# yoshihikoueno/DNNCancerAnnotator

Measured on AMD Instinct MI355X. Metric: MRI slices/sec (fwd+bwd) unet 512x512 bs=8, higher is better.
Workload: dtype f32; 1 GPU; configs/unet.yaml train step (fwd + weighted BCE + bwd + Adam), batch 8 x 512x512x1 per GPU, f32, random-init weights; global_batch=8, parallelism=dp1, kernels=tuned, communicator=False

## Files before the change

### dnncancerannotator_amd/csrc/kernels_mfma.hip

```cpp
#include <stdio.h>
#include <stdlib.h>

#include "fast.h"
#include "kernels.h"
#include "tconv2_dev.h"

namespace dnnca {

typedef float f32x4 __attribute__((ext_vector_type(4)));

static constexpr int TH = 8;
static constexpr int NBUCKET = kPgBuckets;

template <int C, int TW>
struct TG {
    static constexpr int HL = (C + 3) / 4 * 4;
    static constexpr int LEAD = HL - C;
    static constexpr int LS = (LEAD + (TW + 2) * C + 3 + 3) / 4 * 4;
    static constexpr int LS4 = LS / 4;
    static constexpr int N4 = (TH + 2) * LS4;
    static constexpr int npf(int nt) { return (N4 + nt - 1) / nt; }
};

__device__ __forceinline__ void lds_barrier() { asm volatile("s_waitcnt lgkmcnt(0)\n\ts_barrier" ::: "memory"); }
// ... 317 lines not shown
        }
    }
}

__device__ __forceinline__ unsigned long long stamp() {
    unsigned long long t;
    asm volatile("s_memtime %0\n\ts_waitcnt lgkmcnt(0)" : "=s"(t)::"memory");
    return t;
}
#ifdef DNNCA_TUNING
#define STAMP(i)                                                                                        \
    do {                                                                                                \
        if (p.stamps && wave == 0 && lane == 0 && it < 4) p.stamps[((size_t)blockIdx.x * 4 + it) * 8 + (i)] = stamp(); \
    } while (0)
#define STAMP_END(i)                                                                                    \
    do {                                                                                                \
        if (p.stamps && wave == 0 && lane == 0) p.stamps[((size_t)blockIdx.x * 4 + 3) * 8 + (i)] = stamp(); \
    } while (0)
#define DBG_FLAGS(p) ((p).dbg)
#else
#define STAMP(i) do { } while (0)
#define STAMP_END(i) do { } while (0)
#define DBG_FLAGS(p) 0
#endif

struct BwdArgs {
    const float* dz;
    const float* x[2];
    const float* bmat;
    float* dx[2];
    float* slabs[2];
    int acc[2];
    int mask[2];
    int B, H, W;
    int tiles_x, tiles_y;
    float alpha;
    const float* pf_y;
    const float* pf_dpool;
    const unsigned char* pf_idx;
    float pf_alpha;
    const float* tc_in;
    float* tc_din;
    const float* tc_w;
    float* tc_slabs;
    int tc_mask;
    float tc_alpha;
    int dbg;
    unsigned long long* stamps;
};

template <int C, int NSRC, int CO>
struct BW {
    static constexpr int Gw = 12 / CO;
    static constexpr int TW = 32 * Gw;
    static constexpr int CTOT = NSRC * C;
    static constexpr int NPASS = CTOT <= 12 ? 1 : NSRC;
    static constexpr int COd = CTOT / NPASS;
    static constexpr int Gd = (COd == 3 || COd == 6 || COd == 12) ? 12 / COd : (COd == 1 ? 4 : 1);
    static constexpr int WRd = (Gd + 2) * CO, SRd = (WRd + 3) / 4, KSd = 3 * SRd;
    static constexpr int MTX = TW / (16 * Gd);
    static constexpr int WRw = (Gw + 2) * C;
    static constexpr int MROWS = 3 * WRw + 1;
    static constexpr int MT = (MROWS + 15) / 16;
    using TGg = TG<CO, TW>;
    using TGx = TG<C, TW>;
    static constexpr int STAGE4 = TGg::N4 + NSRC * TGx::N4;
    static constexpr int RED4 = NSRC * MT * 256;
    static constexpr int LDS4 = STAGE4 > RED4 ? STAGE4 : RED4;
};

#define DNNCA_DPP_ADD(v, ctrl, rmask) \
    (v) += __builtin_bit_cast(float, __builtin_amdgcn_update_dpp(0, __builtin_bit_cast(int, (v)), (ctrl), (rmask), 0xf, true))
__device__ __forceinline__ float wave_total_l63(float v) {
    DNNCA_DPP_ADD(v, 0x118, 0xf);
    DNNCA_DPP_ADD(v, 0x114, 0xf);
    DNNCA_DPP_ADD(v, 0x112, 0xf);
    DNNCA_DPP_ADD(v, 0x111, 0xf);
    DNNCA_DPP_ADD(v, 0x142, 0xa);
    DNNCA_DPP_ADD(v, 0x143, 0xc);
    return v;
}
__device__ __forceinline__ int slab_index(int mrow, int n);

template <int C, int NSRC, int CO, bool DGRAD, int NT, bool VW = false, bool PF = false, bool TCF = false, bool TCM = false, bool CW = false>
__global__ __launch_bounds__(NT, (VW && NSRC == 1) ? 4 : 1) void k_pgbwd(BwdArgs p) {
    constexpr int NW = NT / 64;
    static_assert(!CW || TCF, "CW is the counted-wait form of the TCF kernel");
    static_assert(!TCF || (VW && NSRC == 2 && C == 3 && CO == 3), "TCF rides in the two-source 3-channel VW kernel");
    static_assert(!TCM || (!VW && !PF && !TCF && NSRC == 2 && DGRAD && C == CO && (C == 6 || C == 12)), "TCM: two-source C -> C conv");
    static_assert(!PF || (NSRC == 1 && C == CO && DGRAD && !VW), "PF: single-source C -> C conv with data gradient");
    static_assert(!VW || (C == 3 && CO == 3 && NT == 512 && DGRAD), "VW: 3 -> 3 channels, eight waves, with data gradient");
    constexpr int NWD = VW ? NW / 2 : NW;
    using Wc = BW<C, NSRC, CO>;
    using TGg = typename Wc::TGg;
    using TGx = typename Wc::TGx;
    constexpr int TW = Wc::TW, Gw = Wc::Gw, Gd = Wc::Gd, COd = Wc::COd, NPASS = Wc::NPASS, SRd = Wc::SRd, KSd = Wc::KSd;
    constexpr int MT = Wc::MT, WRw = Wc::WRw, LSg = TGg::LS, LSx = TGx::LS, Nw = Gw * CO, Nd = Gd * COd;
    static_assert(TW % (16 * Gd) == 0, "tile width must hold whole dgrad M-tiles");
    constexpr int MAIN4 = Wc::LDS4;
    constexpr int PFR = TH / 2 + 2, PFW = Wc::TW / 2 + 2, PFLEAD = (4 - CO % 4) % 4;
    constexpr int PFLS = (PFLEAD + PFW * CO + 3) / 4 * 4, PFN4 = PF ? PFR * PFLS / 4 : 0, PFLI = PFLS / 4, PFNI = PF ? PFR * PFLI : 0;
    constexpr int TCF4 = TCF ? TH * 4 * 24 + 18 : 0;
    constexpr int CIt = 12, KA = 2 * C, KTt = 4 * C, KS1 = KA / 4, MBt = (KTt + 15) / 16;
    constexpr int LWt = Wc::TW / 2, NLP = (TH / 2) * LWt, ROWF = Wc::TW * C;
    constexpr int DT4 = TCM ? TH * ROWF / 4 : 0, XLT4 = TCM ? NLP * CIt / 4 : 0, TCW4 = TCM ? KTt * CIt / 4 : 0;
    static_assert(!TCM || (XLT4 <= NT && LWt % 16 == 0), "TCM: one staging slot per thread, whole M-tiles per input row");
    constexpr int TCM0 = MAIN4 + NW * 48 + 1 + PFN4 + (PFNI + 3) / 4 + TCF4;
    constexpr int DTF = TCM0 * 4, XLTF = DTF + DT4 * 4, TCWF = XLTF + XLT4 * 4;
    constexpr bool TLDS = TCM && C == 12;
    constexpr int TSUM0 = TCM0 + DT4 + XLT4 + TCW4, TSUM4 = TLDS ? NW * MBt * 64 : 0;
    constexpr int DUMP4 = CW ? NT : 0;
    __shared__ float4 lds4[TSUM0 + TSUM4 + DUMP4];
    float* orow = reinterpret_cast<float*>(lds4 + MAIN4) + (threadIdx.x >> 6) * 192;
    float4* dta4 = lds4 + MAIN4 + NW * 48 + 1 + PFN4 + (PFNI + 3) / 4;
    float* tcw = reinterpret_cast<float*>(dta4 + TH * 4 * 24);
    float* pf_dp = reinterpret_cast<float*>(lds4 + MAIN4 + NW * 48 + 1);
    unsigned* pf_ix = reinterpret_cast<unsigned*>(lds4 + MAIN4 + NW * 48 + 1 + PFN4);
    constexpr int NPS = PF ? (PFN4 + NT - 1) / NT : 1;
    static_assert(PFNI == PFN4, "the two pooled tiles have the same number of staging slots");

    const int tid = threadIdx.x, lane = tid & 63, wave = tid >> 6;
    const int m16 = lane & 15, q = lane >> 4, n = m16;
    const int ntiles = p.tiles_x * p.tiles_y * p.B;
    const bool xcd_map = (ntiles & 7) == 0 && (gridDim.x & 7) == 0;

    float* cst = reinterpret_cast<float*>(lds4 + MAIN4 + NW * 48);
    if (threadIdx.x == 0) { cst[0] = 1.0f; cst[1] = 0.0f; }
    if constexpr (TCF) {
        if (threadIdx.x < 72) tcw[threadIdx.x] = p.tc_w[threadIdx.x];
    }
    float tacc[TCF ? 72 : 1], tbias[TCF ? 3 : 1];
#pragma unroll
    for (int i = 0; i < (TCF ? 72 : 1); ++i) tacc[i] = 0.f;
#pragma unroll
    for (int i = 0; i < (TCF ? 3 : 1); ++i) tbias[i] = 0.f;
    const float* ldsf = reinterpret_cast<const float*>(lds4);
    constexpr int CST1 = (MAIN4 + NW * 48) * 4, CST0 = CST1 + 1;
    int offA[MT], stepA[MT];
#pragma unroll
    for (int t = 0; t < MT; ++t) {
        const int mrow = 16 * t + m16;
        if (mrow < 3 * WRw) {
            const int dy = mrow / WRw, j = mrow - dy * WRw;
            offA[t] = dy * LSx + TGx::LEAD + j + q * (Gw * C);
            stepA[t] = 4 * Gw * C;
        } else {
            offA[t] = mrow == 3 * WRw ? CST1 : CST0;
            stepA[t] = 0;
        }
    }
    f32x4 acc[NSRC][MT];
#pragma unroll
    for (int s = 0; s < NSRC; ++s)
#pragma unroll
        for (int t = 0; t < MT; ++t) acc[s][t] = f32x4{0.f, 0.f, 0.f, 0.f};
    constexpr int NWACC = !VW ? 1 : (NSRC == 2 ? 84 : 27);
    float wacc[NWACC];
#pragma unroll
    for (int i = 0; i < NWACC; ++i) wacc[i] = 0.f;

    f32x4 tacc2[TCM ? MBt : 1];
    if constexpr (TCM) {
        if (tid < TCW4) lds4[TCM0 + DT4 + XLT4 + tid] = reinterpret_cast<const float4*>(p.tc_w)[tid];
        if constexpr (TLDS) {
#pragma unroll
            for (int t = 0; t < MBt; ++t) lds4[TSUM0 + (wave * MBt + t) * 64 + lane] = make_float4(0.f, 0.f, 0.f, 0.f);
        }
#pragma unroll
        for (int t = 0; t < MBt; ++t) {
            tacc2[t] = f32x4{0.f, 0.f, 0.f, 0.f};
        }
    }
    if (VW && wave < NWD) __builtin_amdgcn_s_setprio(2);
    float breg[DGRAD ? NPASS * KSd : 1];
    if (DGRAD) {
#pragma unroll
        for (int s = 0; s < NPASS * KSd; ++s) breg[s] = p.bmat[s * 64 + lane];
    }
    const int dxp = n / COd, cod = n % COd;

    float4 preg[TGg::npf(NT)];
    float4 prex[NSRC][TGx::npf(NT)];
    TileMap<CO, TW, NT> mpg;
    TileMap<C, TW, NT> mpx;
    mpg.init(tid, p.W * CO / 4);
    mpx.init(tid, p.W * C / 4);
    float4 prey[PF ? TGg::npf(NT) : 1];
    float4 predp[NPS];
    unsigned preix[NPS];
    auto pf_issue = [&](int b, int x0, int y0) {
        if constexpr (PF) {
            (void)tile_issue<CO, TW, NT>(prey, mpg, p.pf_y, b, x0, y0, p.B, p.H, p.W);
            const int Hp = p.H >> 1, Wp = p.W >> 1, rowf = Wp * CO;
#pragma unroll
            for (int k = 0; k < NPS; ++k) {
                const int id = tid + k * NT;
                const int r = id / PFLI, c4 = id - r * PFLI;
                const int gy = (y0 >> 1) - 1 + r, gf = ((x0 >> 1) - 1) * CO - PFLEAD + 4 * c4;
                const bool ok = id < PFN4 && (unsigned)gy < (unsigned)Hp && gf >= 0 && gf < rowf;
                const size_t off = ok ? ((size_t)b * Hp + gy) * rowf + gf : 0;
                predp[k] = *reinterpret_cast<const float4*>(p.pf_dpool + off);
                if (!ok) predp[k] = make_float4(0.f, 0.f, 0.f, 0.f);
                preix[k] = *reinterpret_cast<const unsigned*>(p.pf_idx + off);
                if (!ok) preix[k] = 0xffffffffu;
            }
        }
    };
    auto pf_commit_pooled = [&]() {
        if constexpr (PF) {
#pragma unroll
            for (int k = 0; k < NPS; ++k) {
                const int id = tid + k * NT;
                if (id < PFN4) {
                    reinterpret_cast<float4*>(pf_dp)[id] = predp[k];
                    pf_ix[id] = preix[k];
                }
            }
        }
    };
    auto pf_transform = [&](unsigned ok) {
        if constexpr (PF) {
            const unsigned char* ixb = reinterpret_cast<const unsigned char*>(pf_ix);
#pragma unroll
            for (int k = 0; k < TGg::npf(NT); ++k) {
                const int r = mpg.row[k], c4 = mpg.c4[k];
                float g[4] = {preg[k].x, preg[k].y, preg[k].z, preg[k].w};
                const float yv[4] = {prey[k].x, prey[k].y, prey[k].z, prey[k].w};
                const bool in = (ok >> k) & 1u;
#pragma unroll
                for (int e = 0; e < 4; ++e) {
                    const int f = 4 * c4 + e - TGg::LEAD;
                    if (in && f >= 0 && f < (TW + 2) * CO) {
                        const int px = f / CO, ch = f - px * CO;
                        const int pr = ((r - 1) >> 1) + 1, pc = ((px - 1) >> 1) + 1;
                        const unsigned pos = (((unsigned)(r - 1) & 1u) << 1) | ((unsigned)(px - 1) & 1u);
                        const int o = PFLEAD + pc * CO + ch;
                        const float dp = ixb[pr * PFLS + o] == pos ? pf_dp[pr * PFLS + o] : 0.f;
                        g[e] = (g[e] + dp) * (yv[e] > 0.f ? 1.0f : p.pf_alpha);
                    }
                }
                preg[k] = make_float4(g[0], g[1], g[2], g[3]);
            }
        }
    };
    unsigned okg = 0, okx = 0;
    auto decode = [&](int t, int& b, int& x0, int& y0) {
        if (xcd_map) t = (t & 7) * (ntiles >> 3) + (t >> 3);
        const int bx = t % p.tiles_x, by = (t / p.tiles_x) % p.tiles_y;
        b = t / (p.tiles_x * p.tiles_y);
        x0 = bx * TW;
        y0 = by * TH;
    };
    int tile = blockIdx.x;
    int it = 0;
    (void)it;
    STAMP(6);
    if (tile < ntiles) {
        int b, x0, y0;
        decode(tile, b, x0, y0);
        okg = tile_issue<CO, TW, NT>(preg, mpg, p.dz, b, x0, y0, p.B, p.H, p.W);
        pf_issue(b, x0, y0);
#pragma unroll
        for (int s = 0; s < NSRC; ++s) okx = tile_issue<C, TW, NT>(prex[s], mpx, p.x[s], b, x0, y0, p.B, p.H, p.W);
    }
    if (DGRAD) {
        asm volatile("s_waitcnt vmcnt(0)" ::: "memory");
#pragma unroll
        for (int s = 0; s < NPASS * KSd; ++s) asm volatile("" : "+v"(breg[s]));
    }

    if constexpr (!CW) {
#define PGBWD_ROLE 0
#include "pgbwd_tiles.h"
#undef PGBWD_ROLE
    } else if (wave < NWD) {
#define PGBWD_ROLE 1
#include "pgbwd_tiles.h"
#undef PGBWD_ROLE
    } else {
#define PGBWD_ROLE 2
#include "pgbwd_tiles.h"
#undef PGBWD_ROLE
        __builtin_amdgcn_s_waitcnt(PG_WAIT_VMCNT0);
    }

    STAMP_END(5);
    if constexpr (VW) {
        float* red = reinterpret_cast<float*>(lds4);
        __syncthreads();
        if (wave >= NWD) {
            const int wv = wave - NWD;
#pragma unroll
            for (int i = 0; i < NWACC; ++i) {
                const float t = wave_total_l63(wacc[i]);
                if (lane == 63 && (NSRC == 2 || wv < 3 || i < 3)) red[NSRC == 2 ? wv * 84 + i : wv * 27 + i] = t;
            }
        } else if constexpr (TCF) {
#pragma unroll
            for (int i = 0; i < 72; ++i) {
                const float t = wave_total_l63(tacc[i]);
                if (lane == 63) red[4 * 84 + wave * 75 + i] = t;
            }
#pragma unroll
            for (int i = 0; i < 3; ++i) {
                const float t = wave_total_l63(tbias[i]);
                if (lane == 63) red[4 * 84 + wave * 75 + 72 + i] = t;
            }
        }
        __syncthreads();
        if constexpr (TCF) {
            if (tid < 75) {
                const float* r2 = red + 4 * 84;
                const float v = (r2[tid] + r2[75 + tid]) + (r2[150 + tid] + r2[225 + tid]);
                const int mrow = tid < 72 ? tid / 6 : tid - 72, col = tid < 72 ? tid % 6 : 6;
                atomicAdd(p.tc_slabs + (size_t)(blockIdx.x % NBUCKET) * 256 + slab_index(mrow, col), v);
            }
        }
        const int bucket = blockIdx.x % NBUCKET;
        for (int i = tid; i < NSRC * 84; i += NT) {
            const int s = i / 84, e = i - s * 84;
            const float v = NSRC == 2 ? red[(2 * s) * 84 + e] + red[(2 * s + 1) * 84 + e] : red[e];
            const int mrow = e < 81 ? (e / 27) * WRw + (e / 3) % 9 : 3 * WRw, co = e < 81 ? e % 3 : e - 81;
            atomicAdd(p.slabs[s] + (size_t)bucket * (MT * 256) + slab_index(mrow, co), v);
        }
        return;
    }
    float* red = reinterpret_cast<float*>(lds4);
    constexpr int PER = NSRC * MT * 256;
    if (NW == 8) {
        if (wave >= 4) {
#pragma unroll
            for (int s = 0; s < NSRC; ++s)
#pragma unroll
                for (int t = 0; t < MT; ++t)
#pragma unroll
                    for (int r = 0; r < 4; ++r) red[(wave - 4) * PER + ((s * MT + t) * 4 + r) * 64 + lane] = acc[s][t][r];
        }
        __syncthreads();
        if (wave < 4) {
#pragma unroll
            for (int s = 0; s < NSRC; ++s)
#pragma unroll
                for (int t = 0; t < MT; ++t)
#pragma unroll
                    for (int r = 0; r < 4; ++r) acc[s][t][r] += red[wave * PER + ((s * MT + t) * 4 + r) * 64 + lane];
        }
        __syncthreads();
    }
    if (wave < 4) {
#pragma unroll
        for (int s = 0; s < NSRC; ++s)
#pragma unroll
            for (int t = 0; t < MT; ++t)
// ... 818 lines not shown
    const int TW = 32 * (12 / CO);
    a.tiles_x = (a.W + TW - 1) / TW;
    a.tiles_y = (a.H + TH - 1) / TH;
    const int ntiles = a.tiles_x * a.tiles_y * B;
    const double bytes = out_bytes + (o.need_din ? 2 : 1) * in_bytes;
    const double fl = (o.need_din ? 2 : 1) * flops;
    if (m->step.pool_fold.conv == &o) {
        auto f3 = pl.first3.find(&o);
        if (f3 != pl.first3.end()) {
            Op* c0 = f3->second;
            const Op& pool = *m->step.pool_fold.pool;
            m->step.pool_fold.conv = nullptr;
            FirstArgs f{};
            f.dskip = o.out.g.p; f.y1 = o.out.d.p;
            f.dpool = pool.out.g.p; f.idx = pool.pool_idx;
            f.x1 = o.inA.d.p; f.xin = c0->inA.d.p;
            f.w = m->p + o.w_off;
            f.pf_alpha = pool.mask_alpha;
            f.mask = o.maskA; f.mask_alpha = o.mask_alpha;
            f.slabs1 = a.slabs[0];
            f.slabs0 = pl.slabs + pl.folds[pl.wslot.find({c0, 0})->second].slab_off;
            f.B = B; f.H = a.H; f.W = a.W;
            const StripGrid sg = strip_grid(B, a.H, a.W, 2048);
            f.nstrips = sg.nstrips; f.nchunks = sg.nchunks;
            const double npx = (double)B * a.H * a.W;
            LAUNCH(m, "first3_bwd", 4.0 * npx * 20.5, 2.0 * npx * (162 + 30),
                   hipLaunchKernelGGL((k_first3<2, 40>), dim3(sg.nblocks), dim3(256), 0, m->stream, f));
            m->step.first_done = c0;
            return true;
        }
    }
    if (!sw.no_bwd3v && o.need_din && C == 3 && CO == 3 && NS == 1 && !o.accA && a.W % 128 == 0 && a.H % TH == 0) {
        const bool pf = m->step.pool_fold.conv == &o;
        double pb = 0.0;
        if (pf) {
            const Op& pool = *m->step.pool_fold.pool;
            m->step.pool_fold.conv = nullptr;
            a.pf_y = o.out.d.p;
            a.pf_dpool = pool.out.g.p;
            a.pf_idx = pool.pool_idx;
            a.pf_alpha = pool.mask_alpha;
            pb = 4.0 * (2 * (double)B * o.out.d.H * o.out.d.W * CO + 2 * (double)B * pool.out.d.H * pool.out.d.W * CO);
        }
        const float* wts = m->p + o.w_off;
        if (a.stamps && pf != sw.stamps_pf) a.stamps = nullptr;
        if (pf) {
            const int g = pg_grid<k_bwd3v<true>, 256>(m, ntiles);
            LAUNCH(m, "bwd3v_pool_3x1_3", bytes + pb, fl, hipLaunchKernelGGL(k_bwd3v<true>, dim3(g), dim3(256), 0, m->stream, a, wts));
        } else {
            const int g = pg_grid<k_bwd3v<false>, 256>(m, ntiles);
#ifdef DNNCA_TUNING
            if (sw.abl == 1) {
                LAUNCH(m, "bwd3v_3x1_3", bytes, fl, hipLaunchKernelGGL((k_bwd3v<false, 1>), dim3(g), dim3(256), 0, m->stream, a, wts));
                return true;
            }
#endif
            LAUNCH(m, "bwd3v_3x1_3", bytes, fl, hipLaunchKernelGGL(k_bwd3v<false>, dim3(g), dim3(256), 0, m->stream, a, wts));
        }
        return true;
    }
    if (m->step.pool_fold.conv == &o) {
        const Op& pool = *m->step.pool_fold.pool;
        m->step.pool_fold.conv = nullptr;
        a.pf_y = o.out.d.p;
        a.pf_dpool = pool.out.g.p;
        a.pf_idx = pool.pool_idx;
        a.pf_alpha = pool.mask_alpha;
        const double pb = 4.0 * (2 * (double)B * o.out.d.H * o.out.d.W * CO + 2 * (double)B * pool.out.d.H * pool.out.d.W * CO);
#define PFX(c)                                                                                                          \
        if (C == c) {                                                                                                   \
            const int g = pg_grid<k_pgbwd<c, 1, c, true, 512, false, true>>(m, ntiles);                                 \
            LAUNCH(m, "pgbwd_pool_" #c "x1_" #c, bytes + pb, fl,                                                        \
                   hipLaunchKernelGGL((k_pgbwd<c, 1, c, true, 512, false, true>), dim3(g), dim3(512), 0, m->stream, a)); \
            return true;                                                                                                \
        }
        PFX(3) PFX(6) PFX(12)
#undef PFX
        return false;
    }
    if (!sw.no_vw && o.need_din && C == 3 && CO == 3 && NS == 2) {
        if (Op* tc = sw.no_tcf ? nullptr : riding_tconv(m, pl, o, 6, a)) {
            const double tb = 4.0 * ((double)B * a.H * a.W * 3 + (double)B * (a.H / 2) * (a.W / 2) * 6);
            if (!sw.pgbwd_old && !a.acc[1] && (size_t)a.H * a.W * 3 * 4 < (size_t)PG_NOWHERE) {
                const int g = pg_grid<k_pgbwd<3, 2, 3, true, 512, true, false, true, false, true>>(m, ntiles);
                LAUNCH(m, "pgbwd_tc_3x2_3", bytes + 2 * tb, fl + 4.0 * B * a.H * a.W * 3 * 6,
                       hipLaunchKernelGGL((k_pgbwd<3, 2, 3, true, 512, true, false, true, false, true>), dim3(g), dim3(512), 0, m->stream, a));
            } else {
                const int g = pg_grid<k_pgbwd<3, 2, 3, true, 512, true, false, true>>(m, ntiles);
                LAUNCH(m, "pgbwd_tc_3x2_3", bytes + 2 * tb, fl + 4.0 * B * a.H * a.W * 3 * 6,
                       hipLaunchKernelGGL((k_pgbwd<3, 2, 3, true, 512, true, false, true>), dim3(g), dim3(512), 0, m->stream, a));
            }
            m->step.tconv_done = tc;
            return true;
        }
        const int g = pg_grid<k_pgbwd<3, 2, 3, true, 512, true>>(m, ntiles);
        LAUNCH(m, "pgbwd_3x2_3", bytes, fl, hipLaunchKernelGGL((k_pgbwd<3, 2, 3, true, 512, true>), dim3(g), dim3(512), 0, m->stream, a));
        return true;
    }
    if (o.need_din && NS == 2 && C == CO && (C == 6 || C == 12) && !sw.no_tcm) {
        if (Op* tc = riding_tconv(m, pl, o, 12, a)) {
            const double tb = 4.0 * ((double)B * a.H * a.W * C + (double)B * (a.H / 2) * (a.W / 2) * 12);
            const double tfl = 4.0 * B * a.H * a.W * C * 12;
#define TCMX(c)                                                                                                         \
            if (C == c) {                                                                                               \
                const int g = pg_grid<k_pgbwd<c, 2, c, true, 512, false, false, false, true>>(m, ntiles);               \
                LAUNCH(m, "pgbwd_tc_" #c "x2_" #c, bytes + 2 * tb, fl + tfl,                                            \
                       hipLaunchKernelGGL((k_pgbwd<c, 2, c, true, 512, false, false, false, true>), dim3(g), dim3(512), 0, m->stream, a)); \
                m->step.tconv_done = tc;                                                                                     \
                return true;                                                                                            \
            }
            TCMX(6) TCMX(12)
#undef TCMX
        }
    }
#define X(c, ns, co)                                                                                            \
    if (C == c && NS == ns && CO == co) {                                                                       \
        if (o.need_din) {                                                                                       \
            const int g = pg_grid<k_pgbwd<c, ns, co, true, 512>>(m, ntiles);                                    \
            LAUNCH(m, "pgbwd_" #c "x" #ns "_" #co, bytes, fl,                                                   \
                   hipLaunchKernelGGL((k_pgbwd<c, ns, co, true, 512>), dim3(g), dim3(512), 0, m->stream, a));   \
        } else {                                                                                                \
            const int g = pg_grid<k_pgbwd<c, ns, co, false, 512>>(m, ntiles);                                   \
            LAUNCH(m, "pgbwd_w_" #c "x" #ns "_" #co, bytes, fl,                                                 \
                   hipLaunchKernelGGL((k_pgbwd<c, ns, co, false, 512>), dim3(g), dim3(512), 0, m->stream, a));  \
        }                                                                                                       \
        return true;                                                                                            \
    }
    CONV_SHAPES(X)
#undef X
    return false;
}

bool fast_pool_fold(Model* m, Op& pool, Op& conv) {
    if (m->sw.no_pool_fold || pool.type != OP_POOL || pool.k != 2 || !pool.pool_idx_valid || !(pool.pool_idx || m->dry)) return false;
    if (!pool.accA || !pool.maskA || pool.mask_alpha != 0.f) return false;
    if (!conv_supported(m, conv) || conv.inB.d.C || !conv.need_din || conv.out.d.p != pool.inA.d.p || !conv.premasked) return false;
    const int C = conv.inA.d.C, CO = conv.out.d.C;
    if (C != CO || !(C == 3 || C == 6 || C == 12)) return false;
    const int TW = 32 * (12 / CO);
    if (!dense(pool.out.g) || !dense(pool.out.d)) return false;
    if ((conv.out.d.W % TW || conv.out.d.H % TH) && !pg_find(m).first3.count(&conv)) return false;
    pool.pool_idx_valid = false;
    m->step.pool_fold.conv = &conv;
    m->step.pool_fold.pool = &pool;
    return true;
}

bool fast_head_in_conv_possible(Model* m) {
    if (m->ops.size() < 2 || !m->head_defer_ok) return false;
    const Op& head = m->ops.back();
    const Op& o = m->ops[m->ops.size() - 2];
    if (head.type != OP_HEAD || !conv_supported(m, o)) return false;
    return o.inA.d.C == 3 && !o.inB.d.C && o.out.d.C == 3 && head.inA.d.p == o.out.d.p && head.inA.d.C == 3 && dense(head.inA.d);
}

template <typename A>
static void head_args(A& a, const Model* m, const Op& head, const float* y, const dnnca_loss_cfg& cfg, float gscale, double n_label) {
    a.hy = y;
    a.hw = m->p + head.w_off; a.hb = m->p + head.b_off;
    a.hpartials = m->head_partials;
    a.hscalars = m->scalars;
    a.hlabel_part = m->step.label_part_valid ? m->label_part : nullptr;
    a.hlabel_nblk = m->step.label_part_nblk;
    a.hcfg = cfg;
    a.hn_label = n_label;
    a.hgscale = gscale;
    a.hmask = head.maskA; a.halpha = head.mask_alpha;
}
static void head_launched(Model* m, const Op& head, int nblocks) {
// ... 253 lines not shown
```

### dnncancerannotator_amd/csrc/model.h

```cpp
#pragma once
#include <initializer_list>
#include <map>
#include <string>
#include <vector>

#include "common.h"
#include "kernels.h"

typedef struct ncclComm* ncclComm_t;

namespace dnnca {

struct OptChunk;

struct T {
    View d, g;
};

inline T tslice(const T& t, int c0, int c) { return T{slice(t.d, c0, c), slice(t.g, c0, c)}; }

enum OpType { OP_CONV = 0, OP_BN, OP_POOL, OP_TCONV, OP_HEAD, OP_JOIN };

struct Op {
    OpType type;
    std::string name;
    T inA, inB, out;
    int64_t w_off = -1, b_off = -1;
    int64_t mm_off = -1, mv_off = -1;
    float alpha = -1.f;
    int k = 0;
    float* nogamma_sum = nullptr;
    bool mean_ready = false;
    bool need_din = true;
    bool accA = false, accB = false;
    bool maskA = false, maskB = false, premasked = false;
    float mask_alpha = 0.f;
    float* coef = nullptr;
    double* ws = nullptr;
    int fused_stats_rows = 0;
    bool elided = false;
    const Op* pool_grad = nullptr;
    bool pool_grad_acc = false;
    bool bwd_sums_rode = false;
    int src_bn[2] = {-1, -1};
    std::vector<int> out_readers;
    unsigned char* pool_idx = nullptr;
    bool pool_idx_valid = false;
};

struct ParamInfo {
    std::string name;
    int64_t shape[4];
    int ndim;
    int trainable;
    int64_t offset;
    int64_t size;
};

struct KStat {
    std::string name;
    int64_t launches = 0;
    double total_ms = 0, bytes = 0, flops = 0;
};

constexpr float kBnMomentum = 0.99f;
constexpr float kBnEps = 1e-3f;

struct RegionState;
struct PgPlan; struct IgPlan; struct Ig3xPlan;

struct ConfThresholds {
    float* dev = nullptr;
    std::vector<int> order;
    int n = 0;
};

struct StepSwitches {
    bool no_fused = false, no_fused_bwd = false, no_first3 = false, no_first3f = false, no_up3f = false, no_tail3 = false;
    bool no_tcf = false, no_tcm = false, no_tconv_ride = false, no_prep_ride = false, no_fold_adam = false, no_pool_fold = false;
    bool no_bwd3v = false, no_vw = false, no_head_in_conv = false, no_label_fusion = false, no_wg_stream = false;
    bool pgbwd_old = false;
    bool fz_up2 = false, fz_all = false, lockstep = false, force_rccl = false;
    std::string fz_only, fzb_only;
    int stamp_c = 0, stamp_ns = 0, stamp_co = 0;
    bool stamps_pf = false;
    int dbg = 0, fzb_dbg = 0, f3f_abl = 0, abl = 0, tail3_variant = 0;
    int nblocks = 0, pg_maxocc = 3;
    int tail3_slots = 2048, tail3_lds = 0;
    int lockstep_maxh = 128;
    int wg_prio = 1;
    size_t bucket_bytes = 8u << 20;
    bool no_join = false;
};
StepSwitches step_switches();

struct StepRequest {
    const float* y = nullptr;
    dnnca_loss_cfg cfg{};
    bool defer_head = false;
    bool head_in_conv = false;
};

struct Model;
struct HostRowRing {
    static constexpr int kAugRing = 4;
    struct Piece { const void* host; size_t bytes; };
    char* dev = nullptr;
    size_t dev_bytes = 0;
    char* pin = nullptr;
    size_t pin_bytes = 0;
    hipEvent_t ev[kAugRing] = {nullptr, nullptr, nullptr, nullptr};
    int k = 0;
    int upload(Model* M, std::initializer_list<Piece> pieces, size_t extra_dev = 0, size_t min_row = 0);
    void release();
};

struct Model {
    dnnca_model_desc desc;
    StepSwitches sw;
    int device = 0;
    hipStream_t stream = nullptr;
    std::vector<ParamInfo> params;
    std::vector<Op> ops;
    std::vector<void*> allocs;
    int64_t nT = 0, nS = 0;
    float *p = nullptr, *g = nullptr, *m = nullptr, *v = nullptr, *state = nullptr;
    double* scalars = nullptr;
    float* out5 = nullptr;
    float *x_stage = nullptr, *y_stage = nullptr, *logits = nullptr, *dlogits = nullptr, *prob = nullptr;
    bool head_defer_ok = false;
    float* y_smooth = nullptr;
    struct RegionLoss { bool on = false; dnnca_region_loss cfg{}; double* ws = nullptr; int sums_batch = 0; } region_loss;
    struct Boundary { float weight = 0.f; float* phi = nullptr; uint32_t* cols = nullptr; int batch = 0, sums_batch = 0; } boundary;
    HostRowRing aug_ring, warp_ring, warpg_ring, affine_ring, intensity_ring;
    float* first_slabs = nullptr;
    static constexpr int kBnTab = 4096;
    double* bn_tab = nullptr;
    float* extra_zero = nullptr;
    size_t extra_zero_n = 0;
    float* nogamma_scratch = nullptr;
    size_t nogamma_n = 0;
    double* join_part = nullptr;
    unsigned* join_ticket = nullptr;
    bool multires() const { return desc.arch == DNNCA_ARCH_MULTIRES; }
    float* head_partials = nullptr;
    double* conf_dev = nullptr;
    T xin;
    int outH = 0, outW = 0;
    int64_t iterations = 0;
    float beta1 = 0.9f, beta2 = 0.999f, eps = 1e-7f;
    int last_batch = 0;
    struct Ema { float* e = nullptr; float decay = 0.f; bool warmup = true; int64_t num_updates = 0; bool in_use = false; } ema;
    float ema_next_om();
    int ema_refuse(const char* what);
    struct Optim {
        bool on = false;
        dnnca_optimizer_cfg cfg{};
        void* table = nullptr;
        OptChunk* chunks = nullptr; int* var_first = nullptr; double* partials = nullptr; double* norms = nullptr; float* scales = nullptr;
        int nchunks = 0, nvars = 0;
        bool norm_clip() const { return on && (cfg.clipnorm > 0.f || cfg.global_clipnorm > 0.f); }
    } opt;
    int opt_launches(float lr, float lr_t, float gscale, float om);
    struct Step {
        struct HeadPending { const float* partials = nullptr; int nblocks = 0, C = 0; float* dw = nullptr; float* dbias = nullptr; } head_pending;
        bool step_init_done = false;
        struct FinalizePending { bool on = false; dnnca_loss_cfg cfg; double n_label = 0, inv_batch_hw = 0; } fin_pending;
        bool head_deferred = false;
        int label_part_nblk = 0; bool label_part_valid = false;
// ... 133 lines not shown
```

### dnncancerannotator_amd/csrc/model.hip

```cpp
#include "abi.h"

#include <rccl/rccl.h>
#include <stdarg.h>
#include <string.h>

#include <algorithm>
#include <cmath>

#include "fast.h"
#include "kernels.h"
#include "optim.h"
#include "region.h"
#include "region_loss.h"
#include "boundary.h"
#include "sens.h"
#include "attr.h"

namespace dnnca {

static thread_local char g_err[1024] = "";

void set_error(const char* fmt, ...) {
    va_list ap;
    va_start(ap, fmt);
    vsnprintf(g_err, sizeof(g_err), fmt, ap);
    va_end(ap);
}

enum { kScalars = 8 };

StepSwitches step_switches() {
    auto on = [](const char* name) { return getenv(name) != nullptr; };
    auto num = [](const char* name, int dflt) { return getenv(name) ? atoi(getenv(name)) : dflt; };
    auto str = [](const char* name) { return std::string(getenv(name) ? getenv(name) : ""); };
    StepSwitches s;
    s.no_fused = on("DNNCA_NO_FUSED");
    s.no_fused_bwd = on("DNNCA_NO_FUSED_BWD");
    s.no_first3 = on("DNNCA_NO_FIRST3");
    s.no_first3f = on("DNNCA_NO_FIRST3F");
    s.no_up3f = on("DNNCA_NO_UP3F");
    s.no_tail3 = on("DNNCA_NO_TAIL3");
    s.no_tcf = on("DNNCA_NO_TCF");
    s.no_tcm = on("DNNCA_NO_TCM");
    s.no_tconv_ride = on("DNNCA_NO_TCONV_RIDE");
    s.no_prep_ride = on("DNNCA_NO_PREP_RIDE");
    s.no_fold_adam = on("DNNCA_NO_FOLD_ADAM");
    s.no_pool_fold = on("DNNCA_NO_POOL_FOLD");
    s.no_bwd3v = on("DNNCA_NO_BWD3V");
    s.no_vw = on("DNNCA_NO_VW");
    s.no_head_in_conv = on("DNNCA_NO_HEAD_IN_CONV");
    s.no_label_fusion = on("DNNCA_NO_LABEL_FUSION");
    s.no_wg_stream = on("DNNCA_NO_WG_STREAM");
    s.pgbwd_old = on("DNNCA_PGBWD_OLD");
    s.fz_up2 = on("DNNCA_FZ_UP2");
    s.fz_all = on("DNNCA_FZ_ALL");
    s.lockstep = on("DNNCA_LOCKSTEP");
    s.force_rccl = on("DNNCA_FORCE_RCCL");
    s.no_join = on("DNNCA_NO_JOIN");
    s.fz_only = str("DNNCA_FZ_ONLY");
    s.fzb_only = str("DNNCA_FZB_ONLY");
    if (sscanf(str("DNNCA_STAMPS").c_str(), "%d,%d,%d", &s.stamp_c, &s.stamp_ns, &s.stamp_co) != 3) s.stamp_c = s.stamp_ns = s.stamp_co = 0;
    s.stamps_pf = on("DNNCA_STAMPS_PF");
    s.dbg = num("DNNCA_DBG", 0);
    s.fzb_dbg = num("DNNCA_FZB_DBG", 0);
    s.f3f_abl = num("DNNCA_F3F_ABL", 0);
    s.abl = num("DNNCA_ABL", 0);
    s.tail3_variant = num("DNNCA_TAIL3_VARIANT", 0);
    s.nblocks = std::max(num("DNNCA_NBLOCKS", 0), 0);
    s.pg_maxocc = num("DNNCA_PG_MAXOCC", 3);
    s.tail3_slots = num("DNNCA_TAIL3_SLOTS", 2048);
    s.tail3_lds = num("DNNCA_TAIL3_LDS", 0);
    s.lockstep_maxh = num("DNNCA_LOCKSTEP_MAXH", 128);
    s.wg_prio = num("DNNCA_WG_PRIO", 1);
    if (const char* e = getenv("DNNCA_BUCKET_BYTES")) s.bucket_bytes = std::max((size_t)atol(e), (size_t)4096);
    return s;
}

static bool head_in_conv_requested(const Model* M, const dnnca_loss_cfg& cfg) {
    return !cfg.label_smoothing && !M->region_loss.on && M->merged_launches() && !M->sw.no_head_in_conv;
}

Model::~Model() {
    region_release(this);
    fast_release(this);
    ig_release(this);
    for (void* a : allocs) (void)hipFree(a);
    if (ema.e) (void)hipFree(ema.e);
    if (opt.table) (void)hipFree(opt.table);
    if (tta_io) (void)hipFree(tta_io);
    if (calib_ws) (void)hipFree(calib_ws);
    for (auto& r : recs) {
        (void)hipEventDestroy(r.a);
        (void)hipEventDestroy(r.b);
    }
    for (auto e : evpool) (void)hipEventDestroy(e);
    if (ev0) (void)hipEventDestroy(ev0);
    if (ev1) (void)hipEventDestroy(ev1);
    if (comm) ncclCommDestroy(comm);
    if (ev_bucket) (void)hipEventDestroy(ev_bucket);
    if (ev_comm_done) (void)hipEventDestroy(ev_comm_done);
    if (comm_stream) (void)hipStreamDestroy(comm_stream);
    for (auto& sl : stage) {
        if (sl.uploaded) (void)hipEventDestroy(sl.uploaded);
        if (sl.done) (void)hipEventDestroy(sl.done);
    }
    if (copy_stream) (void)hipStreamDestroy(copy_stream);
    if (out_ring) (void)hipHostFree(out_ring);
    if (tm_pin) (void)hipHostFree(tm_pin);
    for (HostRowRing* r : {&aug_ring, &warp_ring, &warpg_ring, &affine_ring, &intensity_ring}) r->release();
    if (wg_fork) (void)hipEventDestroy(wg_fork);
    if (wg_join) (void)hipEventDestroy(wg_join);
    if (wg_bucket) (void)hipEventDestroy(wg_bucket);
    if (wg_stream) (void)hipStreamDestroy(wg_stream);
    if (stream) (void)hipStreamDestroy(stream);
}

bool Model::wg_side_begin() {
    const bool off = sw.no_wg_stream;
    if (off || dry || prof_mode == 1 || prof_mode == 3) return false;
    if (!wg_stream) {
        int lo = 0, hi = 0;
        (void)hipDeviceGetStreamPriorityRange(&lo, &hi);
        const int prio = sw.wg_prio == 1 ? lo : (sw.wg_prio == 2 ? hi : 0);
        if (hipStreamCreateWithPriority(&wg_stream, hipStreamNonBlocking, prio) != hipSuccess) { wg_stream = nullptr; return false; }
        if (hipEventCreateWithFlags(&wg_fork, hipEventDisableTiming) != hipSuccess ||
            hipEventCreateWithFlags(&wg_join, hipEventDisableTiming) != hipSuccess ||
            hipEventCreateWithFlags(&wg_bucket, hipEventDisableTiming) != hipSuccess)
            return false;
    }
    if (!wg_fork || !wg_join || !wg_bucket) return false;
    if (hipEventRecord(wg_fork, stream) != hipSuccess || hipStreamWaitEvent(wg_stream, wg_fork, 0) != hipSuccess) return false;
    step.wg_pending = true;
    stream = wg_stream;
    return true;
}

// ... 2289 lines not shown
```

### dnncancerannotator_amd/csrc/pgbwd_tiles.h

```cpp
#pragma unroll 1
    while (tile < ntiles) {
        constexpr int ROLE = PGBWD_ROLE;
        int b, x0, y0;
        decode(tile, b, x0, y0);
        STAMP(0);
        if constexpr (PF) {
            pf_commit_pooled();
            lds_barrier();
            pf_transform(okg);
        }
        if constexpr (CW) {
            float4* dump = lds4 + TSUM0 + TSUM4 + tid;
            tile_commit_all<CO, TW, NT>(preg, okg, lds4, dump, tid);
#pragma unroll
            for (int s = 0; s < NSRC; ++s) tile_commit_all<C, TW, NT>(prex[s], okx, lds4 + TGg::N4 + s * TGx::N4, dump, tid);
        } else {
            tile_commit<CO, TW, NT>(preg, okg, lds4, tid);
#pragma unroll
            for (int s = 0; s < NSRC; ++s) tile_commit<C, TW, NT>(prex[s], okx, lds4 + TGg::N4 + s * TGx::N4, tid);
        }
        lds_barrier();
        constexpr int GOFF = 0, XOFF = TGg::N4 * 4;
        const float* gl = ldsf + GOFF;
        const float* xl = ldsf + XOFF;
        STAMP(1);
        float tin[TCF ? 6 : 1];
        if constexpr (TCF) {
            if (ROLE == 1 || (ROLE == 0 && wave < NWD)) {
                const int pr = lane >> 4, pc = lane & 15;
                const float* ip = p.tc_in + ((((size_t)b * (p.H >> 1) + (y0 >> 1) + pr) * (p.W >> 1)) + (x0 >> 1) + wave * 16 + pc) * 6;
#pragma unroll
                for (int ci = 0; ci < 6; ++ci) tin[ci] = ip[ci];
            }
        }
        float4 txl = make_float4(0.f, 0.f, 0.f, 0.f);
        if constexpr (TCM) {
            if (tid < XLT4) {
                const int r = tid / (LWt * 3), c = tid - r * (LWt * 3);
                txl = reinterpret_cast<const float4*>(p.tc_in)[(((size_t)b * (p.H >> 1) + (y0 >> 1) + r) * (p.W >> 1) + (x0 >> 1)) * 3 + c];
            }
        }
        const int next = tile + gridDim.x;
        if (CW || next < ntiles) {
            int nb, nx0, ny0;
            decode(CW && next >= ntiles ? tile : next, nb, nx0, ny0);
            okg = tile_issue<CO, TW, NT>(preg, mpg, p.dz, nb, nx0, ny0, p.B, p.H, p.W);
            pf_issue(nb, nx0, ny0);
#pragma unroll
            for (int s = 0; s < NSRC; ++s) okx = tile_issue<C, TW, NT>(prex[s], mpx, p.x[s], nb, nx0, ny0, p.B, p.H, p.W);
        }

        STAMP(2);
        if (DGRAD && ROLE != 2 && !(DBG_FLAGS(p) & 1)) {
            constexpr int PERW = Wc::MTX * TH / NWD;
            constexpr int NCH = (VW && NSRC == 1) ? 2 : (PERW >= 4 ? 4 : PERW);
#pragma unroll 1
            for (int j0 = 0; j0 < (ROLE == 0 && VW && wave >= NWD ? 0 : PERW); j0 += NCH) {
#pragma unroll
                for (int ps = 0; ps < NPASS; ++ps) {
                    f32x4 d[NCH];
                    int txs[NCH], tys[NCH];
#pragma unroll
                    for (int i = 0; i < NCH; ++i) {
                        const int t = wave + NWD * (j0 + i);
                        txs[i] = t % Wc::MTX;
                        tys[i] = t / Wc::MTX;
                        d[i] = f32x4{0.f, 0.f, 0.f, 0.f};
                    }
#pragma unroll
                    for (int dy = 0; dy < 3; ++dy)
#pragma unroll
                        for (int k = 0; k < SRd; ++k)
#pragma unroll
                            for (int i = 0; i < NCH; ++i)
                                d[i] = __builtin_amdgcn_mfma_f32_16x16x4f32(
                                    gl[(tys[i] + dy) * LSg + TGg::LEAD + (txs[i] * 16 + m16) * (Gd * CO) + q + 4 * k],
                                    breg[ps * KSd + dy * SRd + k], d[i], 0, 0, 0);
                    constexpr int SPL = (NSRC == 2 && NPASS == 1) ? 2 : 1;
                    constexpr int CS = COd / SPL;
                    constexpr int PER4 = 16 * Gd * CS / 4;
#pragma unroll
                    for (int i = 0; i < NCH; ++i) {
                        const int tx = txs[i], ty = tys[i], y = y0 + ty;
                        if (n < Nd) {
                            const int sp = cod / CS, cs = cod - sp * CS;
#pragma unroll
                            for (int r = 0; r < 4; ++r)
                                orow[sp * (16 * Gd * CS) + (4 * q + r) * (Gd * CS) + dxp * CS + cs] = d[i][r];
                        }
                        __builtin_amdgcn_wave_barrier();
                        const int sp = lane / PER4, i4 = lane - sp * PER4;
                        const int src = NPASS == 2 ? ps : sp;
                        float* dxs;
                        int accs, masks;
                        if constexpr (NPASS == 2) { dxs = ps ? p.dx[1] : p.dx[0]; accs = ps ? p.acc[1] : p.acc[0]; masks = ps ? p.mask[1] : p.mask[0]; }
                        else if constexpr (SPL == 2) { dxs = sp ? p.dx[1] : p.dx[0]; accs = sp ? p.acc[1] : p.acc[0]; masks = sp ? p.mask[1] : p.mask[0]; }
                        else { dxs = p.dx[0]; accs = p.acc[0]; masks = p.mask[0]; }
                        const int f0 = (x0 + tx * 16 * Gd) * C + 4 * i4;
                        if constexpr (CW) {
                            float4 v = reinterpret_cast<const float4*>(orow)[lane < 2 * PER4 ? lane : 0];
                            if (lane < PER4) dta4[(ty * 4 + tx) * 24 + i4] = v;
                            if (p.mask[1]) {
                                const float4 xv = *reinterpret_cast<const float4*>(
                                    xl + (TGx::N4 * 4) + (ty + 1) * LSx + TGx::HL + tx * 16 * Gd * C + 4 * i4);
                                v.x *= xv.x > 0.f ? 1.0f : p.alpha;
                                v.y *= xv.y > 0.f ? 1.0f : p.alpha;
                                v.z *= xv.z > 0.f ? 1.0f : p.alpha;
                                v.w *= xv.w > 0.f ? 1.0f : p.alpha;
                            }
                            const __amdgpu_buffer_rsrc_t rs_dx1 = __builtin_amdgcn_make_buffer_rsrc(
                                (void*)(p.dx[1] + (size_t)b * p.H * p.W * C), 0, p.H * p.W * C * 4, PG_RSRC);
                            const unsigned off = sp == 1 ? ((unsigned)y * (unsigned)(p.W * C) + (unsigned)f0) * 4u : PG_NOWHERE;
                            __builtin_amdgcn_raw_buffer_store_b128(__builtin_bit_cast(pg_u4, v), rs_dx1, off, 0, 0);
                        } else if (TCF && sp == 0) {
                            if (lane < PER4) dta4[(ty * 4 + tx) * 24 + i4] = reinterpret_cast<const float4*>(orow)[lane];
                        } else if (TCM && src == 0) {
                            if (lane < PER4) lds4[TCM0 + (ty * Wc::MTX + tx) * PER4 + i4] = reinterpret_cast<const float4*>(orow)[lane];
                        } else if (lane < SPL * PER4 && f0 < p.W * C && y < p.H) {
                            float4 v = reinterpret_cast<const float4*>(orow)[lane];
                            float* dst = dxs + ((size_t)b * p.H + y) * p.W * C + f0;
                            if (accs) {
                                const float4 o = *reinterpret_cast<const float4*>(dst);
                                v.x += o.x; v.y += o.y; v.z += o.z; v.w += o.w;
                            }
                            if (masks) {
                                const float4 xv = *reinterpret_cast<const float4*>(
                                    xl + src * (TGx::N4 * 4) + (ty + 1) * LSx + TGx::HL + tx * 16 * Gd * C + 4 * i4);
                                v.x *= xv.x > 0.f ? 1.0f : p.alpha;
                                v.y *= xv.y > 0.f ? 1.0f : p.alpha;
                                v.z *= xv.z > 0.f ? 1.0f : p.alpha;
                                v.w *= xv.w > 0.f ? 1.0f : p.alpha;
                            }
                            *reinterpret_cast<float4*>(dst) = v;
                        }
                        __builtin_amdgcn_wave_barrier();
                    }
                }
            }
        }
        if constexpr (TCM) {
            static_assert(Wc::MTX * (16 * Gd * C / 4) == ROWF / 4, "TCM: the M-tiles of a row tile the gradient row");
            if (tid < XLT4) lds4[TCM0 + DT4 + tid] = txl;
            lds_barrier();
            int lo = lane;
            asm volatile("" : "+v"(lo));
            const int m16 = lo & 15, q = lo >> 4;
            int offT[MBt];
#pragma unroll
            for (int t = 0; t < MBt; ++t) {
                const int k = 16 * t + m16, a = k / KA, kr = k - a * KA;
                offT[t] = k < KTt ? DTF + a * ROWF + 2 * q * C + kr : CST0;
            }
            const int boffT = m16 < CIt ? XLTF + q * CIt + m16 : (m16 == CIt ? CST1 : CST0), bstepT = m16 < CIt ? 4 * CIt : 0;
            const int woffT = m16 < CIt ? TCWF + q * CIt + m16 : CST0, wstepT = bstepT;
#pragma unroll 1
            for (int mt = wave; mt < NLP / 16; mt += NW) {
                const int li = mt / (LWt / 16), mx = mt - li * (LWt / 16);
                f32x4 d = f32x4{0.f, 0.f, 0.f, 0.f};
#pragma unroll
                for (int a = 0; a < 2; ++a)
#pragma unroll
                    for (int kk = 0; kk < KS1; ++kk)
                        d = __builtin_amdgcn_mfma_f32_16x16x4f32(ldsf[DTF + (2 * li + a) * ROWF + 2 * (mx * 16 + m16) * C + 4 * kk + q],
                                                                 ldsf[woffT + (a * KS1 + kk) * wstepT], d, 0, 0, 0);
                if (m16 < CIt) {
#pragma unroll
                    for (int r = 0; r < 4; ++r) orow[(4 * q + r) * CIt + m16] = d[r];
                }
                __builtin_amdgcn_wave_barrier();
                if (lane < 16 * CIt / 4) {
                    float4 v = reinterpret_cast<const float4*>(orow)[lane];
                    if (p.tc_mask) {
                        const float4 xv = lds4[TCM0 + DT4 + (li * LWt + mx * 16) * 3 + lane];
                        v.x *= xv.x > 0.f ? 1.0f : p.tc_alpha;
                        v.y *= xv.y > 0.f ? 1.0f : p.tc_alpha;
                        v.z *= xv.z > 0.f ? 1.0f : p.tc_alpha;
                        v.w *= xv.w > 0.f ? 1.0f : p.tc_alpha;
                    }
                    reinterpret_cast<float4*>(p.tc_din)[(((size_t)b * (p.H >> 1) + (y0 >> 1) + li) * (p.W >> 1) + (x0 >> 1) + mx * 16) * 3 + lane] = v;
                }
                __builtin_amdgcn_wave_barrier();
            }
            if constexpr (TLDS) {
#pragma unroll
                for (int t = 0; t < MBt; ++t) tacc2[t] = f32x4{0.f, 0.f, 0.f, 0.f};
            }
#pragma unroll 1
            for (int st = wave; st < NLP / 4; st += NW) {
                const int sd = ((4 * st) / LWt) * 2 * ROWF + ((4 * st) % LWt) * 2 * C;
                const float bv = ldsf[boffT + st * bstepT];
#pragma unroll
                for (int t = 0; t < MBt; ++t)
                    tacc2[t] = __builtin_amdgcn_mfma_f32_16x16x4f32(ldsf[offT[t] + (16 * (t + 1) <= KTt || offT[t] != CST0 ? sd : 0)], bv, tacc2[t], 0, 0, 0);
            }
            if constexpr (TLDS) {
#pragma unroll
                for (int t = 0; t < MBt; ++t) {
                    float4 v = lds4[TSUM0 + (wave * MBt + t) * 64 + lane];
                    v.x += tacc2[t][0]; v.y += tacc2[t][1]; v.z += tacc2[t][2]; v.w += tacc2[t][3];
                    lds4[TSUM0 + (wave * MBt + t) * 64 + lane] = v;
                }
            }
        }
        if constexpr (TCF) {
            if ((ROLE == 1 || (ROLE == 0 && wave < NWD)) && !(DBG_FLAGS(p) & 5)) {
                __builtin_amdgcn_wave_barrier();
                const int pr = lane >> 4, pc = lane & 15;
                const float* dt = reinterpret_cast<const float*>(dta4);
                float din[6] = {0.f, 0.f, 0.f, 0.f, 0.f, 0.f};
#pragma unroll
                for (int a = 0; a < 2; ++a) {
                    float d6[6];
                    const float* rp = dt + (((2 * pr + a) * 4 + wave) * 24) * 4 + (2 * pc) * 3;
#pragma unroll
                    for (int i = 0; i < 6; ++i) d6[i] = rp[i];
#pragma unroll
                    for (int e = 0; e < 2; ++e)
#pragma unroll
                        for (int co = 0; co < 3; ++co) {
// ... 31 lines not shown
                            float xr[2][9], dzv[2][3];
                            auto load = [&](int b, int r) {
#pragma unroll
                                for (int j = 0; j < 9; ++j) xr[b][j] = xb[r * LSx + j];
#pragma unroll
                                for (int co = 0; co < 3; ++co) dzv[b][co] = gb[r * LSg + co];
                            };
                            auto fma27 = [&](int b) {
#pragma unroll
                                for (int j = 0; j < 9; ++j)
#pragma unroll
                                    for (int co = 0; co < 3; ++co) wacc[j * 3 + co] = fmaf(xr[b][j], dzv[b][co], wacc[j * 3 + co]);
                            };
                            load(0, 0);
#pragma unroll 1
                            for (int r = 0; r < TH; r += 2) {
                                load(1, r + 1);
                                fma27(0);
                                load(0, r + 2 < TH ? r + 2 : TH - 1);
                                fma27(1);
                            }
                        } else {
#pragma unroll
                            for (int r = 0; r < TH; ++r)
#pragma unroll
                                for (int co = 0; co < 3; ++co) wacc[co] += gb[r * LSg + co];
                        }
                    }
                } else {
                const int src = wv >> 1;
                const int col = (wv & 1) * 64 + lane;
                constexpr int ROWS = TH;
                const int r0 = 0;
                const float* xb = xl + src * (TGx::N4 * 4) + TGx::LEAD + col * C;
                const float* gb = gl + TGg::HL + col * CO;
                float xw[3][9];
#pragma unroll
                for (int j = 0; j < 9; ++j) { xw[0][j] = xb[r0 * LSx + j]; xw[1][j] = xb[(r0 + 1) * LSx + j]; }
#pragma unroll
                for (int rr = 0; rr < ROWS; ++rr) {
                    const int r = r0 + rr;
                    float dzv[3];
#pragma unroll
                    for (int co = 0; co < 3; ++co) dzv[co] = gb[(r + 1) * LSg + co];
#pragma unroll
                    for (int j = 0; j < 9; ++j) xw[(rr + 2) % 3][j] = xb[(r + 2) * LSx + j];
#pragma unroll
                    for (int dy = 0; dy < 3; ++dy)
#pragma unroll
                        for (int j = 0; j < 9; ++j)
#pragma unroll
                            for (int co = 0; co < 3; ++co)
                                wacc[(dy * 9 + j) * 3 + co] = fmaf(xw[(rr + dy) % 3][j], dzv[co], wacc[(dy * 9 + j) * 3 + co]);
#pragma unroll
                    for (int co = 0; co < 3; ++co) wacc[81 + co] += dzv[co];
                }
                }
            }
        } else {
#pragma unroll 1
        for (int ty = (DBG_FLAGS(p) & 2) ? TH : wave; ty < TH; ty += NW) {
            const int goff = n < Nw ? GOFF + (ty + 1) * LSg + TGg::HL + q * Nw + n : CST0;
            const int gstep = n < Nw ? 4 * Nw : 0;
            int aoffs[NSRC][MT];
#pragma unroll
            for (int s = 0; s < NSRC; ++s)
#pragma unroll
                for (int t = 0; t < MT; ++t)
                    aoffs[s][t] = stepA[t] ? XOFF + s * (TGx::N4 * 4) + ty * LSx + offA[t] : offA[t];
#pragma unroll
            for (int st = 0; st < TW / (4 * Gw); ++st) {
                const float bv = ldsf[goff + st * gstep];
#pragma unroll
                for (int s = 0; s < NSRC; ++s)
#pragma unroll
                    for (int t = 0; t < MT; ++t) {
                        const int ao = 16 * (t + 1) <= 3 * WRw ? aoffs[s][t] + st * (4 * Gw * C) : aoffs[s][t] + st * stepA[t];
                        acc[s][t] = __builtin_amdgcn_mfma_f32_16x16x4f32(ldsf[ao], bv, acc[s][t], 0, 0, 0);
                    }
            }
        }
        }
        STAMP(4);
        lds_barrier();
        STAMP(5);
        ++it;
        tile = next;
    }
```

Measured before the change: 20320 slices/s.

## Double-buffer LDS staging and pair row-segment dx stores in counted-wait pgbwd kernel

Adds a CWX template refinement to the counted-wait TCF backward kernel, on by default as mode 5. DB double-buffers the LDS staging area: commits alternate between two buffers and the end-of-tile barrier is dropped, so the next tile's commit can overlap the current tile's compute. S4 writes two row segments of the second-source gradient per store pass using buffer stores with out-of-bounds suppression, cutting the number of store iterations. The cost is a larger LDS footprint, which may lower occupancy, and more complex sync ordering.

```diff
diff --git a/dnncancerannotator_amd/csrc/kernels_mfma.hip b/dnncancerannotator_amd/csrc/kernels_mfma.hip
--- a/dnncancerannotator_amd/csrc/kernels_mfma.hip
+++ b/dnncancerannotator_amd/csrc/kernels_mfma.hip
@@ -423,10 +423,14 @@
 }
 __device__ __forceinline__ int slab_index(int mrow, int n);
 
-template <int C, int NSRC, int CO, bool DGRAD, int NT, bool VW = false, bool PF = false, bool TCF = false, bool TCM = false, bool CW = false>
+template <int C, int NSRC, int CO, bool DGRAD, int NT, bool VW = false, bool PF = false, bool TCF = false, bool TCM = false, bool CW = false,
+          int CWX = 0>
 __global__ __launch_bounds__(NT, (VW && NSRC == 1) ? 4 : 1) void k_pgbwd(BwdArgs p) {
     constexpr int NW = NT / 64;
     static_assert(!CW || TCF, "CW is the counted-wait form of the TCF kernel");
+    static_assert(!CWX || CW, "CWX refines the counted-wait form");
+    static_assert((CWX & ~5) == 0, "CWX: bits 1 (DB) and 4 (S4)");
+    constexpr bool DB = (CWX & 1) != 0, S4 = (CWX & 4) != 0;
     static_assert(!TCF || (VW && NSRC == 2 && C == 3 && CO == 3), "TCF rides in the two-source 3-channel VW kernel");
     static_assert(!TCM || (!VW && !PF && !TCF && NSRC == 2 && DGRAD && C == CO && (C == 6 || C == 12)), "TCM: two-source C -> C conv");
     static_assert(!PF || (NSRC == 1 && C == CO && DGRAD && !VW), "PF: single-source C -> C conv with data gradient");
@@ -451,7 +455,8 @@
     constexpr bool TLDS = TCM && C == 12;
     constexpr int TSUM0 = TCM0 + DT4 + XLT4 + TCW4, TSUM4 = TLDS ? NW * MBt * 64 : 0;
     constexpr int DUMP4 = CW ? NT : 0;
-    __shared__ float4 lds4[TSUM0 + TSUM4 + DUMP4];
+    constexpr int DB0 = TSUM0 + TSUM4 + DUMP4;
+    __shared__ float4 lds4[DB0 + (DB ? Wc::STAGE4 : 0)];
     float* orow = reinterpret_cast<float*>(lds4 + MAIN4) + (threadIdx.x >> 6) * 192;
     float4* dta4 = lds4 + MAIN4 + NW * 48 + 1 + PFN4 + (PFNI + 3) / 4;
     float* tcw = reinterpret_cast<float*>(dta4 + TH * 4 * 24);
@@ -610,6 +615,8 @@
         for (int s = 0; s < NPASS * KSd; ++s) asm volatile("" : "+v"(breg[s]));
     }
 
+    int cb4 = 0;
+    (void)cb4;
     if constexpr (!CW) {
 #define PGBWD_ROLE 0
 #include "pgbwd_tiles.h"
@@ -1594,9 +1601,21 @@
         if (Op* tc = sw.no_tcf ? nullptr : riding_tconv(m, pl, o, 6, a)) {
             const double tb = 4.0 * ((double)B * a.H * a.W * 3 + (double)B * (a.H / 2) * (a.W / 2) * 6);
             if (!sw.pgbwd_old && !a.acc[1] && (size_t)a.H * a.W * 3 * 4 < (size_t)PG_NOWHERE) {
-                const int g = pg_grid<k_pgbwd<3, 2, 3, true, 512, true, false, true, false, true>>(m, ntiles);
-                LAUNCH(m, "pgbwd_tc_3x2_3", bytes + 2 * tb, fl + 4.0 * B * a.H * a.W * 3 * 6,
-                       hipLaunchKernelGGL((k_pgbwd<3, 2, 3, true, 512, true, false, true, false, true>), dim3(g), dim3(512), 0, m->stream, a));
+                int cwx = sw.pgbwd_cw1 ? 0 : 5;
+#ifdef DNNCA_TUNING
+                if (!sw.pgbwd_cw1 && (sw.pgbwd_cwx == 1 || sw.pgbwd_cwx == 4)) cwx = sw.pgbwd_cwx;
+#endif
+#define CWXV(x)                                                                                                         \
+                if (cwx == x) {                                                                                         \
+                    const int g = pg_grid<k_pgbwd<3, 2, 3, true, 512, true, false, true, false, true, x>>(m, ntiles);   \
+                    LAUNCH(m, "pgbwd_tc_3x2_3", bytes + 2 * tb, fl + 4.0 * B * a.H * a.W * 3 * 6,                       \
+                           hipLaunchKernelGGL((k_pgbwd<3, 2, 3, true, 512, true, false, true, false, true, x>), dim3(g), dim3(512), 0, m->stream, a)); \
+                }
+                CWXV(0) CWXV(5)
+#ifdef DNNCA_TUNING
+                CWXV(1) CWXV(4)
+#endif
+#undef CWXV
             } else {
                 const int g = pg_grid<k_pgbwd<3, 2, 3, true, 512, true, false, true>>(m, ntiles);
                 LAUNCH(m, "pgbwd_tc_3x2_3", bytes + 2 * tb, fl + 4.0 * B * a.H * a.W * 3 * 6,
diff --git a/dnncancerannotator_amd/csrc/model.h b/dnncancerannotator_amd/csrc/model.h
--- a/dnncancerannotator_amd/csrc/model.h
+++ b/dnncancerannotator_amd/csrc/model.h
@@ -80,11 +80,13 @@
     bool no_tcf = false, no_tcm = false, no_tconv_ride = false, no_prep_ride = false, no_fold_adam = false, no_pool_fold = false;
     bool no_bwd3v = false, no_vw = false, no_head_in_conv = false, no_label_fusion = false, no_wg_stream = false;
     bool pgbwd_old = false;
+    bool pgbwd_cw1 = false;
     bool fz_up2 = false, fz_all = false, lockstep = false, force_rccl = false;
     std::string fz_only, fzb_only;
     int stamp_c = 0, stamp_ns = 0, stamp_co = 0;
     bool stamps_pf = false;
     int dbg = 0, fzb_dbg = 0, f3f_abl = 0, abl = 0, tail3_variant = 0;
+    int pgbwd_cwx = 5;
     int nblocks = 0, pg_maxocc = 3;
     int tail3_slots = 2048, tail3_lds = 0;
     int lockstep_maxh = 128;
diff --git a/dnncancerannotator_amd/csrc/model.hip b/dnncancerannotator_amd/csrc/model.hip
--- a/dnncancerannotator_amd/csrc/model.hip
+++ b/dnncancerannotator_amd/csrc/model.hip
@@ -52,6 +52,8 @@
     s.no_label_fusion = on("DNNCA_NO_LABEL_FUSION");
     s.no_wg_stream = on("DNNCA_NO_WG_STREAM");
     s.pgbwd_old = on("DNNCA_PGBWD_OLD");
+    s.pgbwd_cw1 = on("DNNCA_PGBWD_CW1");
+    s.pgbwd_cwx = num("DNNCA_PGBWD_CWX", 5);
     s.fz_up2 = on("DNNCA_FZ_UP2");
     s.fz_all = on("DNNCA_FZ_ALL");
     s.lockstep = on("DNNCA_LOCKSTEP");
diff --git a/dnncancerannotator_amd/csrc/pgbwd_tiles.h b/dnncancerannotator_amd/csrc/pgbwd_tiles.h
--- a/dnncancerannotator_amd/csrc/pgbwd_tiles.h
+++ b/dnncancerannotator_amd/csrc/pgbwd_tiles.h
@@ -9,7 +9,12 @@
             lds_barrier();
             pf_transform(okg);
         }
-        if constexpr (CW) {
+        if constexpr (DB) {
+            float4* dump = lds4 + TSUM0 + TSUM4 + tid;
+            tile_commit_all<CO, TW, NT>(preg, okg, lds4 + cb4, dump, tid);
+#pragma unroll
+            for (int s = 0; s < NSRC; ++s) tile_commit_all<C, TW, NT>(prex[s], okx, lds4 + cb4 + TGg::N4 + s * TGx::N4, dump, tid);
+        } else if constexpr (CW) {
             float4* dump = lds4 + TSUM0 + TSUM4 + tid;
             tile_commit_all<CO, TW, NT>(preg, okg, lds4, dump, tid);
 #pragma unroll
@@ -19,10 +24,11 @@
 #pragma unroll
             for (int s = 0; s < NSRC; ++s) tile_commit<C, TW, NT>(prex[s], okx, lds4 + TGg::N4 + s * TGx::N4, tid);
         }
-        lds_barrier();
+        if constexpr (!DB) lds_barrier();
         constexpr int GOFF = 0, XOFF = TGg::N4 * 4;
         const float* gl = ldsf + GOFF;
         const float* xl = ldsf + XOFF;
+        if constexpr (DB) { gl += cb4 * 4; xl += cb4 * 4; }
         STAMP(1);
         float tin[TCF ? 6 : 1];
         if constexpr (TCF) {
@@ -49,6 +55,7 @@
 #pragma unroll
             for (int s = 0; s < NSRC; ++s) okx = tile_issue<C, TW, NT>(prex[s], mpx, p.x[s], nb, nx0, ny0, p.B, p.H, p.W);
         }
+        if constexpr (DB) lds_barrier();
 
         STAMP(2);
         if (DGRAD && ROLE != 2 && !(DBG_FLAGS(p) & 1)) {
@@ -79,6 +86,41 @@
                     constexpr int SPL = (NSRC == 2 && NPASS == 1) ? 2 : 1;
                     constexpr int CS = COd / SPL;
                     constexpr int PER4 = 16 * Gd * CS / 4;
+                    if constexpr (S4) {
+                        static_assert(NCH == 4 && SPL == 2 && 2 * PER4 <= 64 && 2 * 16 * Gd * CS <= 192, "S4: two row segments fit an orow");
+                        static_assert(VW && 2 * NWD == NW, "S4: the upper half of the output rows is free");
+                        const int e = lane / PER4, i4 = lane - e * PER4;
+                        const __amdgpu_buffer_rsrc_t rs_dx1 = __builtin_amdgcn_make_buffer_rsrc(
+                            (void*)(p.dx[1] + (size_t)b * p.H * p.W * C), 0, p.H * p.W * C * 4, PG_RSRC);
+                        if (n < Nd) {
+                            const int sp = cod / CS, cs = cod - sp * CS;
+#pragma unroll
+                            for (int i = 0; i < NCH; ++i) {
+                                float* dst = sp == 0 ? reinterpret_cast<float*>(dta4 + (tys[i] * 4 + txs[i]) * 24)
+                                                     : orow + (i >> 1) * (NWD * 192) + (i & 1) * (16 * Gd * CS);
+#pragma unroll
+                                for (int r = 0; r < 4; ++r) dst[(4 * q + r) * (Gd * CS) + dxp * CS + cs] = d[i][r];
+                            }
+                        }
+                        __builtin_amdgcn_wave_barrier();
+#pragma unroll
+                        for (int h = 0; h < NCH / 2; ++h) {
+                            const int tx = e == 1 ? txs[2 * h + 1] : txs[2 * h], ty = e == 1 ? tys[2 * h + 1] : tys[2 * h];
+                            const int y = y0 + ty, f0 = (x0 + tx * 16 * Gd) * C + 4 * i4;
+                            float4 v = reinterpret_cast<const float4*>(orow + h * (NWD * 192))[lane < 2 * PER4 ? lane : 0];
+                            if (p.mask[1]) {
+                                const float4 xv = *reinterpret_cast<const float4*>(
+                                    xl + (TGx::N4 * 4) + (ty + 1) * LSx + TGx::HL + tx * 16 * Gd * C + 4 * i4);
+                                v.x *= xv.x > 0.f ? 1.0f : p.alpha;
+                                v.y *= xv.y > 0.f ? 1.0f : p.alpha;
+                                v.z *= xv.z > 0.f ? 1.0f : p.alpha;
+                                v.w *= xv.w > 0.f ? 1.0f : p.alpha;
+                            }
+                            const unsigned off = e < 2 ? ((unsigned)y * (unsigned)(p.W * C) + (unsigned)f0) * 4u : PG_NOWHERE;
+                            __builtin_amdgcn_raw_buffer_store_b128(__builtin_bit_cast(pg_u4, v), rs_dx1, off, 0, 0);
+                        }
+                        __builtin_amdgcn_wave_barrier();
+                    } else {
 #pragma unroll
                     for (int i = 0; i < NCH; ++i) {
                         const int tx = txs[i], ty = tys[i], y = y0 + ty;
@@ -135,6 +177,7 @@
                         }
                         __builtin_amdgcn_wave_barrier();
                     }
+                    }
                 }
             }
         }
@@ -332,6 +375,8 @@
         }
         }
         STAMP(4);
+        if constexpr (DB) cb4 = DB0 - cb4;
+        else
         lds_barrier();
         STAMP(5);
         ++it;
```

Result: no change. 20320 slices/s, median of 2 (+0.0%).
